# tatary/ramses

Measured on AMD Instinct MI355X. Metric: cell-updates/s (Godunov sweep), uniform Sedov3D, higher is better.
Workload: dtype f64

## Files before the change

### include/ramses_amd.h

```cpp
#ifndef RAMSES_AMD_H
#define RAMSES_AMD_H

#include <stddef.h>
#include <stdint.h>

#ifdef __cplusplus
extern "C" {
#endif

#define RAMSES_AMD_OK 0
#define RAMSES_AMD_EINVAL (-1)
#define RAMSES_AMD_EUNSUPPORTED (-2)
#define RAMSES_AMD_EHIP (-3)
#define RAMSES_AMD_ENODEVICE (-4)

enum { RAMSES_AMD_RIEMANN_LLF = 0, RAMSES_AMD_RIEMANN_HLLC = 1,
       RAMSES_AMD_RIEMANN_HLL = 2, RAMSES_AMD_RIEMANN_ACOUSTIC = 3,
       RAMSES_AMD_RIEMANN_EXACT = 4 };
enum { RAMSES_AMD_SCHEME_MUSCL = 0, RAMSES_AMD_SCHEME_PLMDE = 1 };

#define RAMSES_AMD_MAX_NENER 2
#define RAMSES_AMD_MAX_NVAR 16

typedef struct ramses_amd_hydro_params {
// ... 14 lines not shown
  double gamma_rad[RAMSES_AMD_MAX_NENER];
} ramses_amd_hydro_params;

typedef struct ramses_amd_brick {
  int32_t nx, ny, nz;
  int32_t ng;
  int64_t pitch_y;
  int64_t pitch_z;
  int64_t pitch_var;
} ramses_amd_brick;

void ramses_amd_brick_dense(ramses_amd_brick *b, int nx, int ny, int nz, int ng);

const char *ramses_amd_last_error(void);
int ramses_amd_abi_check(size_t sizeof_hydro_params, size_t sizeof_brick);
int ramses_amd_set_device_auto(int world_rank);
int ramses_amd_device_info(char *name, size_t name_len, int *n_cu, size_t *hbm_bytes);

int ramses_amd_godunov_brick(const ramses_amd_hydro_params *p,
                             const ramses_amd_brick *b, const double *d_uold,
                             const double *d_grav, double *d_unew, double dx,
                             double dt, void *stream);

int ramses_amd_godunov_brick_shell(const ramses_amd_hydro_params *p,
                                   const ramses_amd_brick *b, const double *d_uold,
                                   const double *d_grav, double *d_unew, double dx,
                                   double dt, void *stream);
int ramses_amd_godunov_brick_interior(const ramses_amd_hydro_params *p,
                                      const ramses_amd_brick *b, const double *d_uold,
                                      const double *d_grav, double *d_unew, double dx,
                                      double dt, void *stream);

int ramses_amd_godunov_tune(int tile_rows, int zchunk);

int ramses_amd_courant_init(const ramses_amd_hydro_params *p, double dx,
                            double *d_out, void *stream);
int ramses_amd_courant_brick(const ramses_amd_hydro_params *p,
                             const ramses_amd_brick *b, const double *d_uold,
                             const double *d_grav, double dx, double *d_out,
                             void *stream);

int ramses_amd_pdv_brick(const ramses_amd_hydro_params *p, const ramses_amd_brick *b,
                         const double *d_uold, double *d_unew, double dx, double dt,
                         void *stream);

int ramses_amd_fill_ghosts_periodic(const ramses_amd_brick *b, double *d_u,
                                    int nvar, int axes, void *stream);

int64_t ramses_amd_halo_slab_size(const ramses_amd_brick *b, int nvar, int face);
int ramses_amd_halo_pack(const ramses_amd_brick *b, const double *d_u, int nvar,
                         int face, double *d_buf, void *stream);
int ramses_amd_halo_unpack(const ramses_amd_brick *b, double *d_u, int nvar,
                           int face, const double *d_buf, void *stream);

int64_t ramses_amd_mg_workspace_doubles(int level);
int ramses_amd_multigrid_fine_brick(int level, const double *d_rho, double rho_tot,
                                    double fourpi, double epsilon, int *safe_mode,
                                    double *d_phi, double *d_f1, double *d_f2,
                                    double *d_work, int *iters, double *err,
                                    void *stream);
int ramses_amd_gradient_phi_brick(int level, const double *d_phi, double *d_f,
                                  void *stream);
int ramses_amd_mg_gauss_seidel(double *d_phi, const double *d_rhs, int n, double dx2,
                               int redstep, void *stream);
int ramses_amd_mg_residual(const double *d_phi, const double *d_rhs, double *d_res,
                           int n, double dx, double *d_work, double *d_norm2,
// ... 370 lines not shown
```

### ramses_amd/_capi.py

```python
import ctypes as C
import os

HERE = os.path.dirname(os.path.abspath(__file__))
LIB_PATH = os.environ.get("RAMSES_AMD_LIB") or os.path.join(HERE, "lib", "libramses_amd.so")

GAMMA_RAD = 1.33333333334
MAX_NVAR = 16
RIEMANN = {"llf": 0, "hllc": 1, "hll": 2, "acoustic": 3, "exact": 4}
SCHEME = {"muscl": 0, "plmde": 1}


class RamsesAmdError(RuntimeError):
    pass


class HydroParams(C.Structure):
    _fields_ = [
        ("ndim", C.c_int32), ("nvar", C.c_int32),
        ("gamma", C.c_double), ("smallr", C.c_double), ("smallc", C.c_double),
        ("slope_type", C.c_int32), ("riemann", C.c_int32),
        ("slope_theta", C.c_double),
        ("scheme", C.c_int32), ("niter_riemann", C.c_int32),
        ("difmag", C.c_double), ("courant_factor", C.c_double),
        ("fast_math", C.c_int32), ("nener", C.c_int32),
# ... 8 lines not shown
    ]


class RefineCrit(C.Structure):
    _fields_ = [
        ("err_grad_d", C.c_double), ("err_grad_p", C.c_double), ("err_grad_u", C.c_double),
        ("floor_d", C.c_double), ("floor_p", C.c_double), ("floor_u", C.c_double),
        ("n_jeans", C.c_double), ("tail_pix", C.c_double), ("factG", C.c_double),
        ("thr", C.c_double), ("var_cut_refine", C.c_double),
        ("thr_mode", C.c_int32), ("ivar_refine", C.c_int32),
    ]


def make_refine_crit(err_grad_d=-1.0, err_grad_p=-1.0, err_grad_u=-1.0, floor_d=1e-10, floor_p=1e-10, floor_u=1e-10,
                     n_jeans=-1.0, tail_pix=0.0, factG=1.0, thr=0.0, var_cut_refine=-1.0, thr_mode=0, ivar_refine=0):
    return RefineCrit(err_grad_d, err_grad_p, err_grad_u, floor_d, floor_p, floor_u, n_jeans, tail_pix, factG, thr,
                      var_cut_refine, thr_mode, ivar_refine)


_lib = None

_vp, _i, _d, _i64 = C.c_void_p, C.c_int, C.c_double, C.c_int64
_PP, _PB = C.POINTER(HydroParams), C.POINTER(Brick)
SYMBOLS = [
    ("ramses_amd_last_error", C.c_char_p, []),
    ("ramses_amd_abi_check", _i, [C.c_size_t, C.c_size_t]),
    ("ramses_amd_brick_dense", None, [_PB, _i, _i, _i, _i]),
    ("ramses_amd_device_info", _i, [C.c_char_p, C.c_size_t, C.POINTER(C.c_int), C.POINTER(C.c_size_t)]),
    ("ramses_amd_set_device_auto", _i, [_i]),
    ("ramses_amd_godunov_brick", _i, [_PP, _PB, _vp, _vp, _vp, _d, _d, _vp]),
    ("ramses_amd_godunov_brick_shell", _i, [_PP, _PB, _vp, _vp, _vp, _d, _d, _vp]),
    ("ramses_amd_godunov_brick_interior", _i, [_PP, _PB, _vp, _vp, _vp, _d, _d, _vp]),
    ("ramses_amd_godunov_tune", _i, [_i, _i]),
    ("ramses_amd_courant_init", _i, [_PP, _d, _vp, _vp]),
    ("ramses_amd_courant_brick", _i, [_PP, _PB, _vp, _vp, _d, _vp, _vp]),
    ("ramses_amd_pdv_brick", _i, [_PP, _PB, _vp, _vp, _d, _d, _vp]),
    ("ramses_amd_fill_ghosts_periodic", _i, [_PB, _vp, _i, _i, _vp]),
    ("ramses_amd_halo_slab_size", _i64, [_PB, _i, _i]),
    ("ramses_amd_halo_pack", _i, [_PB, _vp, _i, _i, _vp, _vp]),
    ("ramses_amd_halo_unpack", _i, [_PB, _vp, _i, _i, _vp, _vp]),
    ("ramses_amd_mg_workspace_doubles", _i64, [_i]),
    ("ramses_amd_multigrid_fine_brick", _i, [_i, _vp, _d, _d, _d, C.POINTER(C.c_int), _vp, _vp, _vp, _vp,
                                             C.POINTER(C.c_int), C.POINTER(C.c_double), _vp]),
    ("ramses_amd_gradient_phi_brick", _i, [_i, _vp, _vp, _vp]),
    ("ramses_amd_mg_gauss_seidel", _i, [_vp, _vp, _i, _d, _i, _vp]),
    ("ramses_amd_mg_residual", _i, [_vp, _vp, _vp, _i, _d, _vp, _vp, _vp]),
    ("ramses_amd_mg_restrict", _i, [_vp, _vp, _vp, _i, _vp]),
    ("ramses_amd_mg_interp_correct", _i, [_vp, _vp, _i, _vp]),
    ("ramses_amd_mg_smooth_fused", _i, [_vp, _vp, _vp, _vp, _vp, _vp, _i, _d, _i, _vp]),
    ("ramses_amd_mg_tune", _i, [_i]),
    ("ramses_amd_godunov_fine_host", _i, [_PP, _i, _i, _vp, _vp, _i64, _i64, _i, _vp, _vp, _vp, _d, _d]),
    ("ramses_amd_interpol_hydro_brick", _i, [_i, _i, _i, _i, _d, _vp, _vp, _vp]),
    ("ramses_amd_upload_fine_brick", _i, [_i, _i, _i, _d, _vp, _vp, _vp]),
    ("ramses_amd_multigrid_fine_f90", _i, [_i, _i, _vp, _vp, _i64, _i64, _i, _vp, _vp, _d, _d, _d,
                                           C.POINTER(C.c_int), C.POINTER(C.c_int), C.POINTER(C.c_double)]),
    ("ramses_amd_godunov_fine_f90", _i, [_PP, _i, _i, _vp, _vp, _i64, _i64, _i, _vp, _vp, _vp, _i, _d, _d]),
    ("ramses_amd_mg_smooth_fused_ghost", _i, [_vp, _vp, _vp, _vp, _vp, _vp, _i, _i, _i, _i, _d, _i, _vp]),
    ("ramses_amd_godunov_fine_amr_host", _i, [_PP, _i, _i, _vp, _vp, _vp, _vp, _i64, _i64, _vp, _vp, _vp, _vp, _vp, _d, _d, _i, _i, _i]),
    ("ramses_amd_godunov_fine_amr_f90", _i, [_PP, _i, _i, _vp, _vp, _vp, _vp, _i64, _i64, _vp, _vp, _vp, _i, _vp, _vp, _i, _d, _d, _i, _i, _i]),
    ("ramses_amd_godunov_fine_amr_workspace", _i64, [_i, _i64]),
    ("ramses_amd_godunov_fine_amr_device", _i, [_PP, _i, _i, _vp, _vp, _vp, _vp, _i64, _i64, _vp, _vp, _vp, _vp, _vp, _d, _d, _i, _i, _i, _vp, _vp, _vp]),
    ("ramses_amd_halo_multi", _i, [_PB, _vp, _i, _i, _vp, _vp, _vp, _i, _vp]),
    ("ramses_amd_make_boundary_hydro", _i, [_PP, _PB, _vp, _i, _i, _vp, _i, _vp]),
    ("ramses_amd_mg_rhs", _i, [_vp, _vp, _i64, _d, _d, _vp]),
    ("ramses_amd_mg_restrict_ghost", _i, [_vp, _vp, _i, _i, _i, _i, _i, _vp]),
    ("ramses_amd_mg_interp_correct_ghost", _i, [_vp, _i, _i, _i, _i, _vp, _i, _i, _vp, _vp]),
# ... 216 lines not shown
```

### ramses_amd/csrc/capi.hip

```cpp
#include <hip/hip_runtime.h>

#include <cmath>
#include <cstdio>
#include <cstdlib>
#include <cstring>
#include <vector>

#include "../../include/ramses_amd.h"
#include "amr_args.hpp"
#include "amr_sweep_args.hpp"
#include "cg_amr_args.hpp"
#include "mg_amr_args.hpp"
#include "mg_args.hpp"
#include "misc_args.hpp"
#include "pack_args.hpp"
#include "rho_args.hpp"
#include "sweep_args.hpp"
#include "capi_shared.hpp"

using namespace ramses_amd;

static thread_local char g_err[512] = "";
static int g_tile_rows = 0;
static int g_zchunk = 128;
static int g_mg_fused = 1;

static bool is_pow2(double x) {
  if (!(x > 0.0) || !std::isfinite(x)) return false;
  int e;
  return std::frexp(x, &e) == 0.5;
}

static int check_brick(const ramses_amd_brick *b) {
  if (!b) return fail(RAMSES_AMD_EINVAL, "brick is NULL");
  const int nmin = b->ng >= 2 ? 1 : 2;
  if (b->nx < 2 || b->ny < nmin || b->nz < nmin) return fail(RAMSES_AMD_EINVAL, "brick must have >=2 cells per direction, or 1 in y/z with ghost layers (got %d %d %d, ng=%d)", b->nx, b->ny, b->nz, b->ng);
  if (b->ng != 0 && b->ng < 2) return fail(RAMSES_AMD_EINVAL, "ghost width must be 0 or >=2 (got %d)", b->ng);
  if (b->pitch_y < b->nx + 2 * b->ng) return fail(RAMSES_AMD_EINVAL, "pitch_y too small");
  if (b->pitch_z < b->pitch_y * (b->ny + 2 * b->ng)) return fail(RAMSES_AMD_EINVAL, "pitch_z too small");
  if (b->pitch_var < b->pitch_z * (b->nz + 2 * b->ng)) return fail(RAMSES_AMD_EINVAL, "pitch_var too small");
  return 0;
}

extern "C" {

const char *ramses_amd_last_error(void) { return g_err; }
int ramses_amd_set_error(int code, const char *msg) {
  snprintf(g_err, sizeof(g_err), "%s", msg ? msg : "");
  return code;
}

int ramses_amd_abi_check(size_t sizeof_hydro_params, size_t sizeof_brick) {
  if (sizeof_hydro_params != sizeof(ramses_amd_hydro_params) || sizeof_brick != sizeof(ramses_amd_brick))
    return fail(RAMSES_AMD_EINVAL, "ABI mismatch: hydro_params %zu (library %zu), brick %zu (library %zu)",
                sizeof_hydro_params, sizeof(ramses_amd_hydro_params), sizeof_brick, sizeof(ramses_amd_brick));
  return 0;
}
// ... 12 lines not shown
  if (n <= 0) return fail(RAMSES_AMD_ENODEVICE, "no HIP device visible");
  int local = world_rank;
  const char *vars[] = {"OMPI_COMM_WORLD_LOCAL_RANK", "MPI_LOCALRANKID", "PMI_LOCAL_RANK", "SLURM_LOCALID", "LOCAL_RANK"};
  for (const char *v : vars) {
    const char *x = getenv(v);
    if (x && *x) { local = atoi(x); break; }
  }
  if (local < 0) local = 0;
  e = hipSetDevice(local % n);
  if (e != hipSuccess) return hipfail(e, "hipSetDevice");
  return 0;
}

int ramses_amd_device_info(char *name, size_t name_len, int *n_cu, size_t *hbm_bytes) {
  int n = 0;
  hipError_t e = hipGetDeviceCount(&n);
  if (e != hipSuccess || n == 0) return fail(RAMSES_AMD_ENODEVICE, "no HIP device: %s", hipGetErrorString(e));
  hipDeviceProp_t prop;
  int dev = 0;
  hipGetDevice(&dev);
  e = hipGetDeviceProperties(&prop, dev);
  if (e != hipSuccess) return hipfail(e, "hipGetDeviceProperties");
  if (name && name_len) { std::strncpy(name, prop.gcnArchName, name_len - 1); name[name_len - 1] = 0; }
  if (n_cu) *n_cu = prop.multiProcessorCount;
  if (hbm_bytes) *hbm_bytes = prop.totalGlobalMem;
  return n;
}

int ramses_amd_godunov_tune(int tile_rows, int zchunk) {
  if (tile_rows != 0 && tile_rows != 8 && tile_rows != 12) return fail(RAMSES_AMD_EINVAL, "tile_rows must be 8 or 12 (got %d)", tile_rows);
  if (zchunk < 0) return fail(RAMSES_AMD_EINVAL, "zchunk must be >=0");
  g_tile_rows = tile_rows;
  g_zchunk = zchunk ? zchunk : 128;
  return 0;
}

static int check_ndim(const ramses_amd_hydro_params *p, const ramses_amd_brick *b) {
  if (p->ndim < 1 || p->ndim > 3) return fail(RAMSES_AMD_EINVAL, "NDIM must be 1, 2 or 3 (got %d)", p->ndim);
  if (p->ndim < 3 && (b->nz != 1 || b->ng < 2)) return fail(RAMSES_AMD_EINVAL, "NDIM=%d needs a brick with nz=1 and ghost layers (got nz=%d, ng=%d)", p->ndim, b->nz, b->ng);
  if (p->ndim < 2 && b->ny != 1) return fail(RAMSES_AMD_EINVAL, "NDIM=1 needs a brick with ny=nz=1 (got ny=%d)", b->ny);
  return 0;
}

static int godunov_brick_region(const ramses_amd_hydro_params *p, const ramses_amd_brick *b,
                                const double *d_uold, const double *d_grav, double *d_unew,
                                double dx, double dt, int region_first, int region_last, void *stream) {
  if (!p) return fail(RAMSES_AMD_EINVAL, "params is NULL");
  if (int rc = check_brick(b)) return rc;
  if ((unsigned long)b->pitch_z * 8ul >= (1ul << 31) || (unsigned long)b->pitch_var * 8ul >= (1ul << 32))
    return fail(RAMSES_AMD_EUNSUPPORTED,
                "brick of %d x %d x %d cells (+%d ghost layers): a plane of %ld bytes or a variable of %ld bytes is beyond the 32-bit offsets of the "
                "sweep kernel (planes < 2 GiB, variables < 4 GiB): split the level into more bricks (ranks)",
                b->nx, b->ny, b->nz, b->ng, (long)b->pitch_z * 8, (long)b->pitch_var * 8);
  if (!d_uold || !d_unew) return fail(RAMSES_AMD_EINVAL, "uold/unew device pointers are NULL");
  if (d_uold == d_unew) return fail(RAMSES_AMD_EINVAL, "uold and unew must be distinct buffers");
  if (int rc = check_ndim(p, b)) return rc;
  if (int rc = check_nener(p, d_grav != nullptr)) return rc;
  if (int rc = check_nvar(p, "ramses_amd_godunov_brick")) return rc;
  if (p->scheme != RAMSES_AMD_SCHEME_MUSCL && p->scheme != RAMSES_AMD_SCHEME_PLMDE) return fail(RAMSES_AMD_EINVAL, "unknown scheme %d", p->scheme);
  if (p->difmag > 0.0) return fail(RAMSES_AMD_EUNSUPPORTED, "difmag>0 is not implemented on the device yet");
  int slope_type = p->slope_type;
  if (p->ndim == 1 && slope_type == 3) slope_type = 2;
  const bool st1d = slope_type == 4 || slope_type == 5 || slope_type == 6;
  if (st1d && p->ndim != 1)
    return fail(RAMSES_AMD_EUNSUPPORTED, "slope_type=%d exists in NDIM=1 runs of the reference only (0,1,2,3,7,8 in 2-D/3-D)", slope_type);
  if (st1d && (p->nvar != 5 || p->scheme != RAMSES_AMD_SCHEME_MUSCL || d_grav))
    return fail(RAMSES_AMD_EUNSUPPORTED, "slope_type=%d: hydro variables only, scheme='muscl', no gravity", slope_type);
  if (!(slope_type == 0 || slope_type == 1 || slope_type == 2 || slope_type == 3 || slope_type == 7 || slope_type == 8 || st1d))
    return fail(RAMSES_AMD_EUNSUPPORTED, "slope_type=%d is not a slope type of the reference", slope_type);
  if (p->riemann < 0 || p->riemann > 4) return fail(RAMSES_AMD_EINVAL, "unknown Riemann solver %d", p->riemann);
  if (!(dx > 0.0) || !(dt >= 0.0)) return fail(RAMSES_AMD_EINVAL, "dx must be >0 and dt >=0");

  SweepArgs A;
  A.uold = d_uold; A.unew = d_unew; A.grav = d_grav;
  A.nx = b->nx; A.ny = b->ny; A.nz = b->nz; A.ng = b->ng;
  A.pitch_y = b->pitch_y; A.pitch_z = b->pitch_z; A.pitch_var = b->pitch_var;
  A.zchunk = g_zchunk < b->nz ? g_zchunk : b->nz;
  A.dt = dt; A.dx = dx; A.rdx = 1.0 / dx;
  A.P = make_const(p);
  A.pow2 = is_pow2(dx) ? 1 : 0;
  hipStream_t s = reinterpret_cast<hipStream_t>(stream);
  for (int region = region_first; region <= region_last; region++) {
    A.region = region;
    hipError_t e;
    const int nv_hydro = p->nvar > 7 ? 5 + p->nener : p->nvar;
    if (p->nener > 0)
      e = p->fast_math ? fastmode::launch_godunov_sweep_nener(A, slope_type, p->riemann, nv_hydro, p->nener, s)
                       : strictmode::launch_godunov_sweep_nener(A, slope_type, p->riemann, nv_hydro, p->nener, s);
    else
      e = p->fast_math
              ? fastmode::launch_godunov_sweep(A, slope_type, p->riemann, g_tile_rows, p->scheme, nv_hydro, d_grav != nullptr, s)
              : strictmode::launch_godunov_sweep(A, slope_type, p->riemann, g_tile_rows, p->scheme, nv_hydro, d_grav != nullptr, s);
    if (e != hipSuccess) return hipfail(e, "godunov sweep launch");
    if (p->nvar > 7) {
      e = p->fast_math ? fastmode::launch_godunov_sweep_scalars(A, slope_type, p->riemann, g_tile_rows, p->nvar, p->nener, d_grav != nullptr, s)
                       : strictmode::launch_godunov_sweep_scalars(A, slope_type, p->riemann, g_tile_rows, p->nvar, p->nener, d_grav != nullptr, s);
      if (e != hipSuccess) return hipfail(e, "godunov scalar pass launch");
    }
  }
  return 0;
}

int ramses_amd_godunov_brick(const ramses_amd_hydro_params *p, const ramses_amd_brick *b,
                             const double *d_uold, const double *d_grav, double *d_unew,
                             double dx, double dt, void *stream) {
  return godunov_brick_region(p, b, d_uold, d_grav, d_unew, dx, dt, SWEEP_ALL, SWEEP_ALL, stream);
}

int ramses_amd_godunov_brick_shell(const ramses_amd_hydro_params *p, const ramses_amd_brick *b,
                                   const double *d_uold, const double *d_grav, double *d_unew,
// ... 559 lines not shown
```

### ramses_amd/csrc/hydro_sweep.hip

```cpp
#include <hip/hip_runtime.h>

#include <type_traits>

#include "difmag_core.hpp"
#include "hydro_core.hpp"
#include "sweep_args.hpp"

namespace ramses_amd {

#ifdef RAMSES_AMD_FAST
#define SWEEP_NS fastmode
#else
#define SWEEP_NS strictmode
#endif

namespace SWEEP_NS {

constexpr int BX = 64;
#ifndef TILE_SWEEP_BY
#define TILE_SWEEP_BY 12
#endif

template <int BY, int NV>
struct Plane {
  double v[NV][BY][BX];
};

template <int ST, int BY, int NV, bool MASK, bool GRAV, int NX = 0, bool DUTY = false, bool R3 = false, int DPN = 0>
struct Lds {
  static constexpr int NF = NV + NX;
  static constexpr int RING = (ST == 3 || R3) ? 3 : 2;
#ifndef SWEEP_PARK_PLAIN
#ifdef RAMSES_AMD_FAST
#define SWEEP_PARK_PLAIN 1
#else
#define SWEEP_PARK_PLAIN 0
#endif
#endif
  static constexpr bool PARK = MASK || ((GRAV || SWEEP_PARK_PLAIN) && BY == 12);
// ... 59 lines not shown
#ifndef SWEEP_STORE_AUX
#define SWEEP_STORE_AUX 0
#endif
__device__ __forceinline__ double plane_load(const double *var_base, unsigned plane_bytes, unsigned off) {
  __amdgpu_buffer_rsrc_t r = __builtin_amdgcn_make_buffer_rsrc(const_cast<double *>(var_base), 0, BUF_RANGE, 0x00020000);
  return __builtin_bit_cast(double, __builtin_amdgcn_raw_buffer_load_b64(r, off, plane_bytes, 0));
}
__device__ __forceinline__ void plane_store(double *var_base, unsigned plane_bytes, unsigned off, double x) {
  __amdgpu_buffer_rsrc_t r = __builtin_amdgcn_make_buffer_rsrc(var_base, 0, BUF_RANGE, 0x00020000);
  __builtin_amdgcn_raw_buffer_store_b64(__builtin_bit_cast(v2u32, x), r, off, plane_bytes, SWEEP_STORE_AUX);
}

__device__ __forceinline__ int wave_shr1_i(int v) { return __builtin_amdgcn_update_dpp(v, v, 0x138, 0xf, 0xf, false); }
__device__ __forceinline__ int wave_shl1_i(int v) { return __builtin_amdgcn_update_dpp(0, v, 0x130, 0xf, 0xf, true); }
__device__ __forceinline__ int stat_load(const unsigned char *base, unsigned ncell, unsigned lane_cell, unsigned plane_cell) {
  __amdgpu_buffer_rsrc_t r = __builtin_amdgcn_make_buffer_rsrc(const_cast<unsigned char *>(base), 0, ncell, 0x00020000);
  return (int)__builtin_amdgcn_raw_buffer_load_b8(r, lane_cell, plane_cell, 0);
}
__device__ __forceinline__ int dir_load(const int *base, unsigned plane_ints, unsigned col) {
  __amdgpu_buffer_rsrc_t r = __builtin_amdgcn_make_buffer_rsrc(const_cast<int *>(base), 0, BUF_RANGE, 0x00020000);
  return (int)__builtin_amdgcn_raw_buffer_load_b32(r, col * 4u, plane_ints * 4u, 0);
}

template <int NV>
__device__ __forceinline__ void load_uold_cell(const double *uold, long pitch_var, unsigned odd_var, unsigned pb, unsigned off, double (&u)[NV]) {
#pragma unroll
  for (int n = 0; n < NV; n++) u[n] = plane_load(uold + (long)(n & ~1) * pitch_var, pb + (n & 1) * odd_var, off);
}
__device__ __forceinline__ unsigned tile_base_ym(int par, bool inB, unsigned a0, unsigned a1, unsigned b0, unsigned b1) {
  const unsigned a = par ? a1 : a0, b = par ? b1 : b0;
  return inB ? b : a;
}
template <int ST, int RS, int BY, bool GRAV, int SCHEME, int NV, int ROLE, bool MASK, int NE = 0, bool PFIX = false, bool DIFMAG = false>
__device__ __forceinline__ void sweep_march(const SweepArgs &A, unsigned char *smem_raw, const SweepPfix &X = SweepPfix(),
                                            const SweepDifmag &D = SweepDifmag()) {
  static_assert(!PFIX || (MASK && NE == 0 && SCHEME == 0), "pressure_fix: the sweep of a level in tiles, muscl");
  static_assert(!DIFMAG || (MASK && NE == 0 && SCHEME == 0 && !PFIX), "difmag: the sweep of a level in tiles, muscl, no pressure_fix");
  constexpr int NF = NV + (PFIX ? 2 : 0);
  const bool DXPOW2 = A.pow2 != 0;
  constexpr bool DUTY = y_duty<ST, RS, BY, GRAV, SCHEME, NV, MASK, NE, PFIX>();
  static_assert(DUTY || ROLE != ROLE_FULL_LO, "row 2 is a full row like the others unless the y fluxes are shared out");
  constexpr int DPN = DIFMAG ? dif_parked<RS, NV>() : 0;
  typedef Lds<ST, BY, NV, MASK, GRAV, NF - NV, DUTY, DIFMAG, DPN> L;
  double (*dpark)[BY - 4][BX] = reinterpret_cast<double (*)[BY - 4][BX]>(smem_raw + L::dpark_off);
  constexpr int RING = L::RING;
  constexpr bool PARK = L::PARK;
  constexpr int M0 = L::M0;
  Plane<BY, NV> *qring = reinterpret_cast<Plane<BY, NV> *>(smem_raw + L::q_off);
  Plane<L::MR, NF> *mring = reinterpret_cast<Plane<L::MR, NF> *>(smem_raw + L::m_off);
  double (*park)[BY - 4][BX] = reinterpret_cast<double (*)[BY - 4][BX]>(smem_raw + L::park_off);
  double (*yduty)[NF][BX] = reinterpret_cast<double (*)[NF][BX]>(smem_raw + L::duty_off);

  const int tx = threadIdx.x, ty = threadIdx.y;
  const HydroConst &P = A.P;

  const int hb = blockIdx.x;
  int bi = 0;
#pragma unroll
  for (int i = 1; i < 6; i++)
    if (i < A.nbox && hb >= A.box[i].first) bi = i;
  const SweepBox &B = A.box[bi];
  int lb = hb - B.first;
  {
    const int nxcd = 8;
    const int cnt = (bi + 1 < A.nbox ? A.box[bi + 1].first : (int)gridDim.x) - B.first;
    if (cnt % nxcd == 0) {
      const int per = cnt / nxcd;
      lb = (lb % nxcd) * per + lb / nxcd;
    }
  }
#ifndef SWEEP_TILE_YFAST
#define SWEEP_TILE_YFAST 0
#endif
#if SWEEP_TILE_YFAST
  const int tiy = B.ty0 + lb % B.nty;
  const int tix = B.tx0 + (lb / B.nty) % B.ntx;
#else
  const int tix = B.tx0 + lb % B.ntx;
  const int tiy = B.ty0 + (lb / B.ntx) % B.nty;
#endif
  const int tiz = lb / (B.ntx * B.nty);
  int x0 = tix * (BX - 4);
  int y0 = tiy * (BY - 4);
  int z0 = B.zlo + tiz * B.zchunk;
  int z1 = min(z0 + B.zchunk, B.zhi);
  if (MASK) {
    const int4 w = reinterpret_cast<const int4 *>(A.work)[hb];
    x0 = w.x; y0 = w.y; z0 = w.z; z1 = w.w;
  }

  const int xu = x0 - 2 + tx;
  const int yu = y0 - 2 + ty;
  int xi, yi;
  if (A.ng == 0) {
    xi = xu < 0 ? xu + A.nx : (xu >= A.nx ? xu - A.nx : xu);
    xi = xi >= A.nx ? xi % A.nx : xi;
    yi = yu < 0 ? yu + A.ny : (yu >= A.ny ? yu - A.ny : yu);
    yi = yi >= A.ny ? yi % A.ny : yi;
  } else {
    xi = min(max(xu, -A.ng), A.nx + A.ng - 1) + A.ng;
    yi = min(max(yu, -A.ng), A.ny + A.ng - 1) + A.ng;
  }
  const unsigned colb = (unsigned)(xi + yi * (int)A.pitch_y) * 8u;
  int tyu = 0, yis = 0, xa = 0, tA = 0, tB = 0, drow = 0;
  bool inB = false;
  unsigned *sloc = reinterpret_cast<unsigned *>(smem_raw + L::sloc_off);
  if (MASK) {
    tyu = __builtin_amdgcn_readfirstlane(ty);
    const int ys = y0 - 2 + tyu;
    yis = ys < 0 ? ys + A.ny : (ys >= A.ny ? ys - A.ny : ys);
    const int xs = x0 - 2;
    xa = xs < 0 ? xs + A.nx : xs;
    tA = xa >> 6; tB = tA + 1 < A.ntx ? tA + 1 : 0;
    inB = (xa & 63) + tx >= 64;
    drow = A.ntx * (yis >> 3);
    const int lind = (xi & 1) + 2 * (yis & 1);
    sloc[ty * BX + tx] = ((unsigned)((long)lind * A.ngd) + (unsigned)(((xi >> 1) & (TILE_OX - 1)) + TILE_OX * ((yis >> 1) & (TILE_OY - 1)))) * 8u;
  }
  const double *__restrict__ uold = A.uold;
  double *__restrict__ unew = A.unew;
  const double *__restrict__ grav = A.grav;

#ifndef SWEEP_LATE_BASE
// ... 477 lines not shown
      }
#pragma unroll
      for (int n = 0; n < NF; n++) {
        if (PARK) { park[n][ty - 2][tx] = px[n]; if (!y_give) park[NF + n][ty - 2][tx] = fy[n]; }
        else { partx[n] = px[n]; fyown[n] = fy[n]; }
      }
      {
        const unsigned pb = MASK ? zpart(c - 1) * 8u : plane_off(c - 1);
        const unsigned so = (c >= z0 + 1) ? (MASK ? ((r_upd && (ok_zlo & CELL_OWNED)) ? tbp(c - 1) : BUF_OOB) : colb_upd) : BUF_OOB;
#pragma unroll
        for (int n = 0; n < NV; n++) {
          if (MASK) plane_store(unew + (long)(n & ~1) * A.pitch_var, pb + (n & 1) * odd_var, so, un[n]);
          else plane_store(unew + (long)n * A.pitch_var, pb, so, un[n]);
        }
        if constexpr (PFIX) { plane_store(X.divu, pb, so, un[NV]); plane_store(X.enew, pb, so, un[NV + 1]); }
      }
      if constexpr (LATE) { if (MASK) load_base(c, bcar); else load_u(c, bcar); }
    }
    if (RING == 3) { const int t = sa; sa = sb; sb = sc; sc = t; }
    else { const int t = sa; sa = sb; sb = t; }
    if (MASK) ok_zlo = okc;
    if (TRIM) rinv_c = rinv_n;
#if SWEEP_CYCLE_PROBE
    pr_a += pr_t1 - pr_t0; pr_w += pr_t2 - pr_t1; pr_b += __builtin_readcyclecounter() - pr_t2; pr_n += 1;
#endif
  }
#if SWEEP_CYCLE_PROBE
  if (tx == 0 && blockIdx.x < PROBE_BLOCKS && ty < PROBE_ROWS) {
    unsigned long long *o = sweep_cycle_probe[blockIdx.x][ty];
    o[0] = pr_a; o[1] = pr_w; o[2] = pr_b; o[3] = pr_n; o[4] = (unsigned long long)ty;
    o[5] = (unsigned long long)__builtin_amdgcn_s_getreg((31 << 11) | 4);
  }
#endif
}

template <int ST, int RS, int BY, bool GRAV, int SCHEME, int NV, bool MASK = false>
__global__ __launch_bounds__(BX *BY) void godunov_sweep_kernel(SweepArgs A) {
  extern __shared__ __attribute__((aligned(16))) unsigned char smem_raw[];
  const int ty = threadIdx.y;
  if (ty >= 2 && ty <= BY - 3) __builtin_amdgcn_s_setprio(3);
  if (ty == 0) sweep_march<ST, RS, BY, GRAV, SCHEME, NV, ROLE_HALO, MASK>(A, smem_raw);
  else if (ty == BY - 1) sweep_march<ST, RS, BY, GRAV, SCHEME, NV, ROLE_HALO_HI, MASK>(A, smem_raw);
  else if (ty == 1) sweep_march<ST, RS, BY, GRAV, SCHEME, NV, ROLE_LOW, MASK>(A, smem_raw);
  else if (ty == BY - 2) sweep_march<ST, RS, BY, GRAV, SCHEME, NV, ROLE_HIGH, MASK>(A, smem_raw);
  else {
    if constexpr (y_duty<ST, RS, BY, GRAV, SCHEME, NV, MASK>()) {
      if (ty == 2) { sweep_march<ST, RS, BY, GRAV, SCHEME, NV, ROLE_FULL_LO, MASK>(A, smem_raw); return; }
    }
    sweep_march<ST, RS, BY, GRAV, SCHEME, NV, ROLE_FULL, MASK>(A, smem_raw);
  }
}

#ifndef RAMSES_AMD_FAST
template <int ST, int NV>
struct PfixRows {
  static constexpr int BY = (ST == 3 && NV == 7) ? 6 : 8;
};
template <int ST, int RS, int BY, bool GRAV, int NV>
__global__ __launch_bounds__(BX *BY) void godunov_sweep_pfix_kernel(SweepArgs A, SweepPfix X) {
  extern __shared__ __attribute__((aligned(16))) unsigned char smem_raw[];
  static_assert(Lds<ST, BY, NV, true, GRAV, 2>::bytes <= 160 * 1024, "the pressure_fix sweep fits one workgroup's LDS");
  const int ty = threadIdx.y;
  if (ty >= 2 && ty <= BY - 3) __builtin_amdgcn_s_setprio(3);
  if (ty == 0) sweep_march<ST, RS, BY, GRAV, 0, NV, ROLE_HALO, true, 0, true>(A, smem_raw, X);
  else if (ty == BY - 1) sweep_march<ST, RS, BY, GRAV, 0, NV, ROLE_HALO_HI, true, 0, true>(A, smem_raw, X);
  else if (ty == 1) sweep_march<ST, RS, BY, GRAV, 0, NV, ROLE_LOW, true, 0, true>(A, smem_raw, X);
// ... 629 lines not shown
    B.tx0 = tx0; B.ntx = tx1 - tx0; B.ty0 = ty0; B.nty = ty1 - ty0;
    B.zlo = zlo; B.zhi = zhi; B.zchunk = zchunk < (zhi - zlo) ? zchunk : (zhi - zlo);
    B.first = nblocks;
    nblocks += B.ntx * B.nty * ((zhi - zlo + B.zchunk - 1) / B.zchunk);
  };
  const int zc = A.zchunk;
  if (A.region == SWEEP_ALL || (A.region == SWEEP_SHELL && !splittable)) {
    add_box(0, NTX, 0, NTY, 0, A.nz, zc);
  } else if (A.region == SWEEP_INTERIOR) {
    if (splittable) add_box(1, NTX - 1, 1, NTY - 1, zb, A.nz - zb, zc);
  } else if (A.region == SWEEP_SHELL) {
    const int zs = 32;
    add_box(0, 1, 1, NTY - 1, zb, A.nz - zb, zs);
    add_box(NTX - 1, NTX, 1, NTY - 1, zb, A.nz - zb, zs);
    add_box(0, NTX, 0, 1, zb, A.nz - zb, zs);
    add_box(0, NTX, NTY - 1, NTY, zb, A.nz - zb, zs);
    add_box(0, NTX, 0, NTY, 0, zb, zs);
    add_box(0, NTX, 0, NTY, A.nz - zb, A.nz, zs);
  } else {
    return -1;
  }
  if (nblocks == 0) return 0;
  A.nblocks = nblocks;
  return nblocks;
}

static bool tile_items(SweepArgs &A) {
  if (!A.stat || !A.dir || !A.work || A.ng != 0 || A.nwork <= 0) return false;
  A.nblocks = A.nwork;
  A.nbox = 1;
  return true;
}

template <int ST, int RS, int BY, bool GRAV, int SCHEME, int NV, bool MASK>
static hipError_t launch_sweep(const SweepArgs &A, hipStream_t s) {
  if constexpr (!sweep_variant(ST, RS, BY, GRAV, SCHEME, NV, MASK)) {
    return hipErrorInvalidValue;
  } else {
    typedef Lds<ST, BY, NV, MASK, GRAV, 0, y_duty<ST, RS, BY, GRAV, SCHEME, NV, MASK>()> L;
    static_assert(L::bytes <= 160 * 1024, "one workgroup's LDS");
    return launch_kernel(godunov_sweep_kernel<ST, RS, BY, GRAV, SCHEME, NV, MASK>, dim3(A.nblocks), dim3(BX, BY), L::bytes, s, A);
  }
}
template <int ST>
hipError_t SweepOf<ST>::sweep(SweepArgs &A, int rs, int by, int scheme, int nvar, bool grav, hipStream_t s) {
  return pick(rs, Solvers(), [&](auto r) {
    constexpr int RS = decltype(r)::value;
    const bool tiles = A.stat != nullptr;
    const int rows = sweep_rows(ST, RS, nvar, scheme, tiles);
    if (by == 0 || rows == 8) by = rows;
    const int planned = plan_boxes(A, by);
    if (planned < 0) return hipErrorInvalidValue;
    if (planned == 0) return hipSuccess;
    if (tiles) {
      if (!tile_items(A)) return hipErrorInvalidValue;
    } else if (!is_1d(ST) && nvar == 5 && scheme != 1) {
      scheme = 0;
    }
    return pick(by, IntList<8, 12, TILE_SWEEP_BY>(), [&](auto b) { return pick(nvar, Nvars(), [&](auto nv) { return pick(scheme, Schemes(), [&](auto sc) {
      return pick(grav, [&](auto g) { return pick(tiles, [&](auto m) {
        return launch_sweep<ST, RS, decltype(b)::value, decltype(g)::value, decltype(sc)::value, decltype(nv)::value, decltype(m)::value>(A, s);
      }); }); }); }); });
  });
}

#ifndef RAMSES_AMD_FAST
template <int ST>
hipError_t SweepOf<ST>::pfix(SweepArgs &A, const SweepPfix &X, int rs, int nvar, bool grav, hipStream_t s) {
  if (!X.divu || !X.enew || !tile_items(A)) return hipErrorInvalidValue;
  A.box[0] = SweepBox{0, 1, 0, 1, 0, A.nz, A.nz, 0};
  return pick_variant(SolversOf<ST>(), rs, nvar, grav, [&](auto r, auto nv, auto g) {
    constexpr int RS = decltype(r)::value, NV = decltype(nv)::value, BY = PfixRows<ST, NV>::BY;
    constexpr bool GRAV = decltype(g)::value;
// ... 166 lines not shown
```

### ramses_amd/csrc/sweep_args.hpp

```cpp
#pragma once
#include "hydro_core.hpp"

namespace ramses_amd {

enum { SWEEP_ALL = 0, SWEEP_INTERIOR = 1, SWEEP_SHELL = 2 };

enum { CELL_REFINED = 1, CELL_OWNED = 2, CELL_GHOST = 4 };
constexpr int TILE_OX = 32, TILE_OY = 4, TILE_OZ = 4, TILE_OCTS = TILE_OX * TILE_OY * TILE_OZ;

struct SweepBox {
  int tx0, ntx, ty0, nty, zlo, zhi, zchunk, first;
};

struct SweepArgs {
  const double *uold;
  double *unew;
  const double *grav;
  const unsigned char *stat = nullptr;
  const int *dir = nullptr;
  const int *work = nullptr;
  int ntx = 0, nty = 0, ntz = 0, nwork = 0;
  int base_uold = 0;
  long ngd = 0, ncoarse = 0;
  int nx, ny, nz;
  int ng;
  long pitch_y, pitch_z, pitch_var;
  int zchunk;
  int region;
  int nbox, nblocks;
  SweepBox box[6];
  double dt, dx, rdx;
  int pow2;
  HydroConst P;
};

struct SweepPfix {
  double *divu = nullptr, *enew = nullptr;
};

struct SweepDifmag {
  double difmag = 0.0;
};

struct SurfArgs {
  const double *uold = nullptr, *grav = nullptr;
  const unsigned char *stat = nullptr;
  const int *dir = nullptr, *tileid = nullptr;
  const int *events = nullptr;
  const int *ig = nullptr;
  double *rec = nullptr;
  int nevent = 0;
  long base = 0, ncoarse = 0, ngd = 0, ncell = 0;
  int no = 0, ntx = 0, nty = 0, ntz = 0;
  double dt = 0, dx = 0, rdx = 0;
  int pow2 = 0;
  int qminor = 0;
  HydroConst P;
};

namespace strictmode {
hipError_t launch_godunov_sweep_nener(SweepArgs &A, int slope_type, int riemann, int nvar, int nener, hipStream_t s);
hipError_t launch_godunov_sweep_scalars(SweepArgs &A, int slope_type, int riemann, int by, int nvar, int nener, bool grav, hipStream_t s);
hipError_t launch_surface_flux(const SurfArgs &A, int slope_type, int riemann, int nvar, int scheme, bool grav, hipStream_t s);
hipError_t launch_godunov_sweep(SweepArgs &A, int slope_type, int riemann, int by, int scheme, int nvar,
                                bool grav, hipStream_t s);
int tile_sweep_rows(int riemann, int nvar, int slope_type, int scheme);
// ... 18 lines not shown
```

### ramses_amd/hydro.py

```python
import ctypes as C

import torch

from . import _capi
from ._capi import check, lib


def _ptr(t):
    return C.c_void_p(t.data_ptr()) if t is not None else None


def _stream():
    return C.c_void_p(torch.cuda.current_stream().cuda_stream)


def godunov_tune(tile_rows=0, zchunk=0):
    check(lib().ramses_amd_godunov_tune(int(tile_rows), int(zchunk)))


class HydroLevel:

    def __init__(self, nx, ny, nz, dx, params=None, ng=0, device="cuda", poisson=False, bound_type=None,
                 bound_state=None, no_inflow=False):
        if not torch.cuda.is_available():
            raise _capi.RamsesAmdError("HydroLevel needs a GPU (torch.cuda.is_available() is False); "
                                       "there is no CPU fallback")
        self.params = params if params is not None else _capi.make_params()
        self.nx, self.ny, self.nz, self.ng, self.dx = nx, ny, nz, ng, float(dx)
        self.nvar = self.params.nvar
        self.brick = _capi.dense_brick(nx, ny, nz, ng)
        shape = (self.nvar, nz + 2 * ng, ny + 2 * ng, nx + 2 * ng)
        self.device = torch.device(device)
        self.uold = torch.zeros(shape, dtype=torch.float64, device=self.device)
        self.unew = torch.zeros(shape, dtype=torch.float64, device=self.device)
        self.f = None
        if poisson:
            self.f = torch.zeros((3,) + shape[1:], dtype=torch.float64, device=self.device)
        self._red = torch.zeros(4, dtype=torch.float64, device=self.device)
        self.dtnew = 0.0
        self._dt_swept = None
        self.bound_type = dict(bound_type or {})
        self.bound_state = dict(bound_state or {})
        self.no_inflow = bool(no_inflow)
        if self.bound_type and ng < 2:
            raise _capi.RamsesAmdError("physical boundaries need ghost layers (ng >= 2)")
        for face in (0, 2, 4):
            if (face in self.bound_type) != (face + 1 in self.bound_type):
                raise _capi.RamsesAmdError("a direction is either periodic or has a boundary on both faces")
        self._periodic_axes = sum(1 << a for a in range(3) if 2 * a not in self.bound_type)

# ... 73 lines not shown
```

Measured before the change: 46.37 billion.

## Add persistent-workgroup sweep plan with full-column tiles and split remainder

Adds a persistent-kernel mode for the Godunov sweep. By default one workgroup per CU loops over tiles, marching full z columns, and the remainder tiles are split into z pieces chosen by a cost model. This replaces the fixed zchunk decomposition and is meant to cut per-block priming overhead from repeated z-chunk starts and to balance tail work. It adds a __syncthreads between segments and may lose latency hiding, because fewer workgroups are resident than in the chunked launch.

Result: slower. 45.85 billion (-1.1%).

```diff
diff --git a/include/ramses_amd.h b/include/ramses_amd.h
--- a/include/ramses_amd.h
+++ b/include/ramses_amd.h
@@ -70,6 +70,8 @@
                                       double dt, void *stream);
 
 int ramses_amd_godunov_tune(int tile_rows, int zchunk);
+
+int ramses_amd_godunov_persist(int workgroups);
 
 int ramses_amd_courant_init(const ramses_amd_hydro_params *p, double dx,
                             double *d_out, void *stream);
diff --git a/ramses_amd/_capi.py b/ramses_amd/_capi.py
--- a/ramses_amd/_capi.py
+++ b/ramses_amd/_capi.py
@@ -64,6 +64,7 @@
     ("ramses_amd_godunov_brick_shell", _i, [_PP, _PB, _vp, _vp, _vp, _d, _d, _vp]),
     ("ramses_amd_godunov_brick_interior", _i, [_PP, _PB, _vp, _vp, _vp, _d, _d, _vp]),
     ("ramses_amd_godunov_tune", _i, [_i, _i]),
+    ("ramses_amd_godunov_persist", _i, [_i]),
     ("ramses_amd_courant_init", _i, [_PP, _d, _vp, _vp]),
     ("ramses_amd_courant_brick", _i, [_PP, _PB, _vp, _vp, _d, _vp, _vp]),
     ("ramses_amd_pdv_brick", _i, [_PP, _PB, _vp, _vp, _d, _d, _vp]),
diff --git a/ramses_amd/csrc/capi.hip b/ramses_amd/csrc/capi.hip
--- a/ramses_amd/csrc/capi.hip
+++ b/ramses_amd/csrc/capi.hip
@@ -23,6 +23,8 @@
 static thread_local char g_err[512] = "";
 static int g_tile_rows = 0;
 static int g_zchunk = 128;
+static bool g_zchunk_set = false;
+static int g_persist = 0;
 static int g_mg_fused = 1;
 
 static bool is_pow2(double x) {
@@ -101,7 +103,29 @@
   if (zchunk < 0) return fail(RAMSES_AMD_EINVAL, "zchunk must be >=0");
   g_tile_rows = tile_rows;
   g_zchunk = zchunk ? zchunk : 128;
-  return 0;
+  g_zchunk_set = zchunk > 0;
+  return 0;
+}
+
+int ramses_amd_godunov_persist(int workgroups) {
+  if (workgroups < -1) return fail(RAMSES_AMD_EINVAL, "workgroups must be -1 (chunked plan), 0 (one per CU) or > 0 (got %d)", workgroups);
+  g_persist = workgroups;
+  return 0;
+}
+
+static int persist_workgroups() {
+  static int env_on = -1;
+  if (env_on < 0) { const char *e = getenv("RAMSES_AMD_SWEEP_PERSIST"); env_on = !(e && e[0] == '0'); }
+  if (!env_on || g_zchunk_set || g_persist < 0) return 0;
+  if (g_persist > 0) return g_persist;
+  static int cus[64] = {0};
+  int dev = 0;
+  if (hipGetDevice(&dev) != hipSuccess || dev < 0 || dev >= 64) return 0;
+  if (cus[dev] == 0) {
+    int n = 0;
+    cus[dev] = (hipDeviceGetAttribute(&n, hipDeviceAttributeMultiprocessorCount, dev) == hipSuccess && n > 0) ? n : -1;
+  }
+  return cus[dev] > 0 ? cus[dev] : 0;
 }
 
 static int check_ndim(const ramses_amd_hydro_params *p, const ramses_amd_brick *b) {
@@ -145,6 +169,7 @@
   A.nx = b->nx; A.ny = b->ny; A.nz = b->nz; A.ng = b->ng;
   A.pitch_y = b->pitch_y; A.pitch_z = b->pitch_z; A.pitch_var = b->pitch_var;
   A.zchunk = g_zchunk < b->nz ? g_zchunk : b->nz;
+  A.persist_g = (region_first == SWEEP_SHELL || p->nener > 0) ? 0 : persist_workgroups();
   A.dt = dt; A.dx = dx; A.rdx = 1.0 / dx;
   A.P = make_const(p);
   A.pow2 = is_pow2(dx) ? 1 : 0;
diff --git a/ramses_amd/csrc/hydro_sweep.hip b/ramses_amd/csrc/hydro_sweep.hip
--- a/ramses_amd/csrc/hydro_sweep.hip
+++ b/ramses_amd/csrc/hydro_sweep.hip
@@ -5,6 +5,7 @@
 #include "difmag_core.hpp"
 #include "hydro_core.hpp"
 #include "sweep_args.hpp"
+#include "sweep_plan.hpp"
 
 namespace ramses_amd {
 
@@ -130,8 +131,8 @@
   return inB ? b : a;
 }
 template <int ST, int RS, int BY, bool GRAV, int SCHEME, int NV, int ROLE, bool MASK, int NE = 0, bool PFIX = false, bool DIFMAG = false>
-__device__ __forceinline__ void sweep_march(const SweepArgs &A, unsigned char *smem_raw, const SweepPfix &X = SweepPfix(),
-                                            const SweepDifmag &D = SweepDifmag()) {
+__device__ __forceinline__ void sweep_segment(const SweepArgs &A, unsigned char *smem_raw, const SweepPfix &X, const SweepDifmag &D,
+                                              const int x0, const int y0, const int z0, const int z1) {
   static_assert(!PFIX || (MASK && NE == 0 && SCHEME == 0), "pressure_fix: the sweep of a level in tiles, muscl");
   static_assert(!DIFMAG || (MASK && NE == 0 && SCHEME == 0 && !PFIX), "difmag: the sweep of a level in tiles, muscl, no pressure_fix");
   constexpr int NF = NV + (PFIX ? 2 : 0);
@@ -152,41 +153,6 @@
   const int tx = threadIdx.x, ty = threadIdx.y;
   const HydroConst &P = A.P;
 
-  const int hb = blockIdx.x;
-  int bi = 0;
-#pragma unroll
-  for (int i = 1; i < 6; i++)
-    if (i < A.nbox && hb >= A.box[i].first) bi = i;
-  const SweepBox &B = A.box[bi];
-  int lb = hb - B.first;
-  {
-    const int nxcd = 8;
-    const int cnt = (bi + 1 < A.nbox ? A.box[bi + 1].first : (int)gridDim.x) - B.first;
-    if (cnt % nxcd == 0) {
-      const int per = cnt / nxcd;
-      lb = (lb % nxcd) * per + lb / nxcd;
-    }
-  }
-#ifndef SWEEP_TILE_YFAST
-#define SWEEP_TILE_YFAST 0
-#endif
-#if SWEEP_TILE_YFAST
-  const int tiy = B.ty0 + lb % B.nty;
-  const int tix = B.tx0 + (lb / B.nty) % B.ntx;
-#else
-  const int tix = B.tx0 + lb % B.ntx;
-  const int tiy = B.ty0 + (lb / B.ntx) % B.nty;
-#endif
-  const int tiz = lb / (B.ntx * B.nty);
-  int x0 = tix * (BX - 4);
-  int y0 = tiy * (BY - 4);
-  int z0 = B.zlo + tiz * B.zchunk;
-  int z1 = min(z0 + B.zchunk, B.zhi);
-  if (MASK) {
-    const int4 w = reinterpret_cast<const int4 *>(A.work)[hb];
-    x0 = w.x; y0 = w.y; z0 = w.z; z1 = w.w;
-  }
-
   const int xu = x0 - 2 + tx;
   const int yu = y0 - 2 + ty;
   int xi, yi;
@@ -730,6 +696,84 @@
     o[5] = (unsigned long long)__builtin_amdgcn_s_getreg((31 << 11) | 4);
   }
 #endif
+}
+
+constexpr bool sweep_persist(int RS, int BY, int NV, bool GRAV, bool MASK, int NE) {
+#ifdef RAMSES_AMD_FAST
+  constexpr bool fast = true;
+#else
+  constexpr bool fast = false;
+#endif
+  return !MASK && NE == 0 && (BY == 12 ? (fast && RS == RIEMANN_LLF) : (RS != RIEMANN_EXACT && NV <= 6 && !(NV == 6 && GRAV)));
+}
+#ifndef SWEEP_TILE_YFAST
+#define SWEEP_TILE_YFAST 0
+#endif
+
+template <int BY>
+__device__ __forceinline__ void sweep_chunk_of_block(const SweepArgs &A, const int hb, int &x0, int &y0, int &z0, int &z1) {
+  int bi = 0;
+#pragma unroll
+  for (int i = 1; i < 6; i++)
+    if (i < A.nbox && hb >= A.box[i].first) bi = i;
+  const SweepBox &B = A.box[bi];
+  int lb = hb - B.first;
+  {
+    const int nxcd = 8;
+    const int cnt = (bi + 1 < A.nbox ? A.box[bi + 1].first : (int)gridDim.x) - B.first;
+    if (cnt % nxcd == 0) {
+      const int per = cnt / nxcd;
+      lb = (lb % nxcd) * per + lb / nxcd;
+    }
+  }
+#if SWEEP_TILE_YFAST
+  const int tiy = B.ty0 + lb % B.nty;
+  const int tix = B.tx0 + (lb / B.nty) % B.ntx;
+#else
+  const int tix = B.tx0 + lb % B.ntx;
+  const int tiy = B.ty0 + (lb / B.ntx) % B.nty;
+#endif
+  const int tiz = lb / (B.ntx * B.nty);
+  x0 = tix * (BX - 4);
+  y0 = tiy * (BY - 4);
+  z0 = B.zlo + tiz * B.zchunk;
+  z1 = min(z0 + B.zchunk, B.zhi);
+}
+
+template <int ST, int RS, int BY, bool GRAV, int SCHEME, int NV, int ROLE, bool MASK, int NE = 0, bool PFIX = false, bool DIFMAG = false>
+__device__ __forceinline__ void sweep_march(const SweepArgs &A, unsigned char *smem_raw, const SweepPfix &X = SweepPfix(),
+                                            const SweepDifmag &D = SweepDifmag()) {
+  const int hb = blockIdx.x;
+  if constexpr (sweep_persist(RS, BY, NV, GRAV, MASK, NE)) {
+    for (int s = 0;; s++) {
+      int x0, y0, z0, z1;
+      if (A.plan_g > 0) {
+        const SweepBox &B = A.box[0];
+        int tile;
+        if (!sweepplan::segment(B.ntx * B.nty, B.zlo, B.zhi, A.plan_g, A.plan_k, hb, s, tile, z0, z1)) return;
+#if SWEEP_TILE_YFAST
+        const int tiy = B.ty0 + tile % B.nty, tix = B.tx0 + tile / B.nty;
+#else
+        const int tix = B.tx0 + tile % B.ntx, tiy = B.ty0 + tile / B.ntx;
+#endif
+        x0 = tix * (BX - 4);
+        y0 = tiy * (BY - 4);
+        if (s > 0) __syncthreads();
+      } else {
+        sweep_chunk_of_block<BY>(A, hb, x0, y0, z0, z1);
+      }
+      sweep_segment<ST, RS, BY, GRAV, SCHEME, NV, ROLE, MASK, NE, PFIX, DIFMAG>(A, smem_raw, X, D, x0, y0, z0, z1);
+      if (A.plan_g <= 0) return;
+    }
+  } else {
+    int x0, y0, z0, z1;
+    sweep_chunk_of_block<BY>(A, hb, x0, y0, z0, z1);
+    if (MASK) {
+      const int4 w = reinterpret_cast<const int4 *>(A.work)[hb];
+      x0 = w.x; y0 = w.y; z0 = w.z; z1 = w.w;
+    }
+    sweep_segment<ST, RS, BY, GRAV, SCHEME, NV, ROLE, MASK, NE, PFIX, DIFMAG>(A, smem_raw, X, D, x0, y0, z0, z1);
+  }
 }
 
 template <int ST, int RS, int BY, bool GRAV, int SCHEME, int NV, bool MASK = false>
@@ -1425,13 +1469,25 @@
   return true;
 }
 
+static void plan_persistent(SweepArgs &A, bool kernel_can) {
+  A.plan_g = A.plan_k = 0;
+  if (!kernel_can || A.persist_g <= 0 || A.nbox != 1 || !(A.region == SWEEP_ALL || A.region == SWEEP_INTERIOR)) return;
+  const SweepBox &B = A.box[0];
+  if (B.zhi - B.zlo >= sweepplan::MAX_NZ) return;
+  const sweepplan::Plan P = sweepplan::make(B.ntx * B.nty, B.zhi - B.zlo, A.persist_g);
+  if (P.g <= 0) return;
+  A.plan_g = P.g; A.plan_k = P.k;
+  A.nblocks = P.g;
+}
+
 template <int ST, int RS, int BY, bool GRAV, int SCHEME, int NV, bool MASK>
-static hipError_t launch_sweep(const SweepArgs &A, hipStream_t s) {
+static hipError_t launch_sweep(SweepArgs &A, hipStream_t s) {
   if constexpr (!sweep_variant(ST, RS, BY, GRAV, SCHEME, NV, MASK)) {
     return hipErrorInvalidValue;
   } else {
     typedef Lds<ST, BY, NV, MASK, GRAV, 0, y_duty<ST, RS, BY, GRAV, SCHEME, NV, MASK>()> L;
     static_assert(L::bytes <= 160 * 1024, "one workgroup's LDS");
+    plan_persistent(A, sweep_persist(RS, BY, NV, GRAV, MASK, 0));
     return launch_kernel(godunov_sweep_kernel<ST, RS, BY, GRAV, SCHEME, NV, MASK>, dim3(A.nblocks), dim3(BX, BY), L::bytes, s, A);
   }
 }
diff --git a/ramses_amd/csrc/sweep_args.hpp b/ramses_amd/csrc/sweep_args.hpp
--- a/ramses_amd/csrc/sweep_args.hpp
+++ b/ramses_amd/csrc/sweep_args.hpp
@@ -32,6 +32,8 @@
   double dt, dx, rdx;
   int pow2;
   HydroConst P;
+  int persist_g = 0;
+  int plan_g = 0, plan_k = 0;
 };
 
 struct SweepPfix {
diff --git a/ramses_amd/csrc/sweep_plan.hpp b/ramses_amd/csrc/sweep_plan.hpp
--- /dev/null
+++ b/ramses_amd/csrc/sweep_plan.hpp
@@ -0,0 +1,61 @@
+#pragma once
+
+namespace ramses_amd {
+namespace sweepplan {
+
+#if defined(__HIPCC__)
+#define SWEEP_PLAN_FN __host__ __device__ inline
+#else
+#define SWEEP_PLAN_FN inline
+#endif
+
+constexpr int SEG_COST = 3;
+constexpr int SEG_PRIMING = 2;
+constexpr int MIN_PIECE = 8;
+constexpr int NXCD = 8;
+constexpr int MAX_NZ = 1 << 16;
+
+struct Plan {
+  int g, k;
+};
+
+SWEEP_PLAN_FN int ceil_div(int a, int b) { return (a + b - 1) / b; }
+
+SWEEP_PLAN_FN long remainder_cost(int R, int nz, int G, int k) { return (long)ceil_div(R * k, G) * (ceil_div(nz, k) + SEG_COST); }
+
+SWEEP_PLAN_FN Plan make(int T, int nz, int G) {
+  Plan P = {0, 1};
+  if (T <= 0 || nz <= 0 || G <= 0) return P;
+  const int full = T / G, R = T - full * G;
+  if (R > 0) {
+    const int kmax = nz / MIN_PIECE > 1 ? nz / MIN_PIECE : 1;
+    long best = remainder_cost(R, nz, G, 1);
+    for (int k = 2; k <= kmax; k++) {
+      const long c = remainder_cost(R, nz, G, k);
+      if (c < best) { best = c; P.k = k; }
+    }
+  }
+  P.g = full > 0 ? G : (R * P.k < G ? R * P.k : G);
+  return P;
+}
+
+SWEEP_PLAN_FN int slot_of(int g, int w) { return g % NXCD == 0 ? (w % NXCD) * (g / NXCD) + w / NXCD : w; }
+
+SWEEP_PLAN_FN bool segment(int T, int zlo, int zhi, int g, int k, int w, int s, int &tile, int &z0, int &z1) {
+  const int full = T / g, R = T - full * g;
+  const int slot = slot_of(g, w);
+  if (s < full) {
+    tile = s * g + slot; z0 = zlo; z1 = zhi;
+    return true;
+  }
+  const int i = (s - full) * g + slot;
+  if (i >= R * k) return false;
+  const int p = i / R, nz = zhi - zlo;
+  tile = full * g + (i - p * R);
+  z0 = zlo + p * nz / k;
+  z1 = zlo + (p + 1) * nz / k;
+  return true;
+}
+
+}
+}
diff --git a/ramses_amd/hydro.py b/ramses_amd/hydro.py
--- a/ramses_amd/hydro.py
+++ b/ramses_amd/hydro.py
@@ -16,6 +16,10 @@
 
 def godunov_tune(tile_rows=0, zchunk=0):
     check(lib().ramses_amd_godunov_tune(int(tile_rows), int(zchunk)))
+
+
+def godunov_persist(workgroups=0):
+    check(lib().ramses_amd_godunov_persist(int(workgroups)))
 
 
 class HydroLevel:
```
